# google/yggdrasil-decision-forests

Measured on NVIDIA H100. Metric: GBT boosting iters/sec, 10M rows x 200 num feats, higher is better.
Workload: dtype int64 fixed-point sums (q24 gradients), f64 split scores

## Files before the change

yggdrasil-decision-forests_b200/_build.py:

```python
import os
import subprocess

HERE = os.path.dirname(os.path.abspath(__file__))
CSRC = os.path.join(HERE, "csrc")
LIB = os.environ.get("YGG_B200_LIB") or os.path.join(HERE, "libygg_b200.so")
EXTRA_FLAGS = os.environ.get("YGG_B200_NVCC_FLAGS", "").split()
SOURCES = ["ygg_engine.cu", "ygg_dataspec.cc", "ygg_model_io.cc", "ygg_comm.cc", "ygg_binning.cu"]
HEADERS = ["ygg_device.cuh", "ygg_kernels.cuh", "../../include/ygg_b200.h",
           "../../include/ygg_b200_dataspec.h", "../../include/ygg_b200_model.h", "ygg_hist.cuh", "ygg_hist_seg.cuh", "ygg_wide.cuh", "ygg_presort.cuh",
           "../../include/ygg_b200_comm.h", "ygg_internal.h"]

NVCC_FLAGS = [
    "-gencode", "arch=compute_90a,code=sm_90a", "-O3", "-lineinfo", "-std=c++17",
    "-Xcompiler", "-fPIC", "-shared", "-ldl",
]


def _nvcc():
    for cand in (os.environ.get("NVCC"), "/usr/local/cuda/bin/nvcc", "nvcc"):
        if cand and (os.path.sep not in cand or os.path.exists(cand)):
            return cand
    return "nvcc"


def stale():
    if not os.path.exists(LIB):
        return True
    t = os.path.getmtime(LIB)
    for f in SOURCES + HEADERS:
        p = os.path.join(CSRC, f)
        if os.path.exists(p) and os.path.getmtime(p) > t:
            return True
    return False


def build(force=False, verbose=False):
    if os.environ.get("YGG_B200_LIB") and os.path.exists(LIB) and not force:
        return LIB
    if not force and not stale():
        return LIB
    srcs = [os.path.join(CSRC, s) for s in SOURCES if os.path.exists(os.path.join(CSRC, s))]
    import fcntl
    with open(LIB + ".lock", "w") as lock:
        fcntl.flock(lock, fcntl.LOCK_EX)
        try:
            if not force and not stale():
                return LIB
            tmp = "%s.%d.tmp" % (LIB, os.getpid())
            cmd = [_nvcc()] + NVCC_FLAGS + EXTRA_FLAGS + (["-Xptxas", "-v"] if verbose else []) + ["-o", tmp] + srcs
            subprocess.check_call(cmd)
            os.replace(tmp, LIB)
        finally:
            fcntl.flock(lock, fcntl.LOCK_UN)
    return LIB


if __name__ == "__main__":
    print(build(force=True, verbose=True))
```

yggdrasil-decision-forests_b200/csrc/ygg_engine.cu:

```cuda
#include <algorithm>
#include <mutex>
#include <random>
#include <cmath>
#include <cstdarg>
#include <cstdio>
#include <cstdlib>
#include <cstring>
#include <limits>
#include <map>
#include <queue>
#include <string>
#include <thread>
#include <vector>

#include <cuda_runtime.h>
#include <cub/device/device_radix_sort.cuh>
#include <cub/device/device_scan.cuh>
#include <nvtx3/nvToolsExt.h>

#include "../../include/ygg_b200.h"
#include "ygg_internal.h"
#include "../../include/ygg_b200_model.h"
#include "ygg_kernels.cuh"
#include "ygg_wide.cuh"
// ... 43 lines not shown
  if (static_cast<int>(done.size()) <= device) done.resize(device + 1, 0);
  if (done[device]) return;
  cudaMemPool_t pool;
  if (cudaDeviceGetDefaultMemPool(&pool, device) == cudaSuccess) {
    unsigned long long threshold = ~0ull;
    cudaMemPoolSetAttribute(pool, cudaMemPoolAttrReleaseThreshold, &threshold);
  }
  cudaGetLastError();
  done[device] = 1;
}

template <typename T>
int dev_alloc(T** p, size_t count) {
  int device = 0;
  cudaGetDevice(&device);
  configure_pool_once(device);
  const size_t bytes = std::max<size_t>(count, 1) * sizeof(T);
  YGG_CUDA(cudaMallocAsync(reinterpret_cast<void**>(p), bytes, nullptr));
  YGG_CUDA(cudaMemsetAsync(*p, 0, bytes, nullptr));
  YGG_CUDA(cudaStreamSynchronize(nullptr));
  return YGG_OK;
}
template <typename T>
int dev_alloc_plain(T** p, size_t count) {
  YGG_CUDA(cudaMalloc(reinterpret_cast<void**>(p), std::max<size_t>(count, 1) * sizeof(T)));
  return YGG_OK;
}
inline void dev_free(void* p) {
  if (p != nullptr) cudaFreeAsync(p, nullptr);
}

struct ProfileSlot {
  double ms = 0;
  int64_t launches = 0;
};

}


struct LossRec {
  double loss_sum;
  unsigned long long correct;
};

enum ShardMode { kShardNone = 0, kShardFeatures = 1, kShardRows = 2 };

struct HistLaunch {
  int mode;
  int G, S;
  int chunk, grid;
  int window, passes;
  int FL, T;
  int SL;
};

struct ygg_gbt {
  ygg_dataset* ds = nullptr;
  ygg_gbt_config cfg{};
  cudaStream_t stream = nullptr;
  bool has_labels = false;
  uint8_t* d_label_u8 = nullptr;
  float* d_label_f32 = nullptr;
  float initial_prediction = 0.f;
  float* d_pred = nullptr;
  float* d_g = nullptr;
  float* d_h = nullptr;
  uint32_t* d_q24 = nullptr;
  uint32_t* d_hq24 = nullptr;
  uint2* d_act = nullptr;
  uint32_t* d_act_h = nullptr;
  int32_t* d_act_count = nullptr;
  int32_t* d_act_sub = nullptr;
  uint32_t* d_root_cnt = nullptr;
  bool root_cnt_valid = false;
  int n_blocks = 0;
  uint16_t* d_node_of_row = nullptr;
  DeviceState* d_st = nullptr;
  LevelDesc* d_levels = nullptr;
  Family* d_fam[2] = {nullptr, nullptr};
  int32_t* d_slot_node[2] = {nullptr, nullptr};
  NodeRec* d_nodes_all = nullptr;
  NodeRec* d_nodes_scratch = nullptr;
  int tree_capacity = 0;
  unsigned long long* d_hist_sum[2] = {nullptr, nullptr};
  uint32_t* d_hist_cnt[2] = {nullptr, nullptr};
  unsigned long long* d_hist_hsum[2] = {nullptr, nullptr};
  Candidate* d_cand = nullptr;
  uint32_t* d_cand_mask = nullptr;
  int64_t wide_total = 0;
  int wide_slots = 0;
  bool counted = false;
  unsigned long long* d_wsum = nullptr;
  uint32_t* d_wcnt = nullptr;
  unsigned long long* d_whsum = nullptr;
  unsigned long long* d_wnode_sum[2] = {nullptr, nullptr};
  uint32_t* d_wnode_cnt[2] = {nullptr, nullptr};
  unsigned long long* d_wnode_hsum[2] = {nullptr, nullptr};
  float* d_wide_thr = nullptr;
  int32_t* d_wide_feature = nullptr;
  int32_t* d_wide_bins = nullptr;
  int set_words = 0;
  int64_t sort_total = 0;
  int64_t* d_sort_off = nullptr;
  int32_t* d_wide_cat = nullptr;
  int32_t* d_wide_na_bin = nullptr;
  uint32_t* d_wide_set = nullptr;
// ... 265 lines not shown
  cudaFuncAttributes fa{};
  YGG_CUDA(cudaFuncGetAttributes(&fa, k_hist<false, kHistPacked>));
  *budget = static_cast<size_t>(optin) - fa.sharedSizeBytes;
  return YGG_OK;
}
constexpr size_t kHist2SmemBudget = 216 * 1024;

int sub_blocks_of(const ygg_gbt* h) { return h->ds->n_pad / kBlockRows >= 512 ? 8 : 1; }
int chunk_max_count(ygg_gbt* h, int chunk_blocks, uint32_t** d_sub, uint32_t* out_max) {
  const int kSubBlocks = sub_blocks_of(h);
  const ygg_dataset* ds = h->ds;
  const int f_count = h->hist_f_end - h->hist_f_begin;
  const int n_blocks = static_cast<int>(ds->n_pad / kBlockRows);
  const int n_subs = (n_blocks + kSubBlocks - 1) / kSubBlocks;
  if (*d_sub == nullptr) {
    YGG_RETURN_IF_ERROR(dev_alloc(d_sub, static_cast<size_t>(n_subs) * f_count * kMaxBins + 1));
    k_sub_counts<<<dim3(n_subs, f_count), 256>>>(ds->d_bins, ds->n, ds->n_pad, h->hist_f_begin, kSubBlocks, *d_sub);
    YGG_RETURN_IF_ERROR(check_launch("k_sub_counts"));
  }
  uint32_t* d_max = *d_sub + static_cast<size_t>(n_subs) * f_count * kMaxBins;
  YGG_CUDA(cudaMemset(d_max, 0, sizeof(uint32_t)));
  const int subs_per_chunk = chunk_blocks / kSubBlocks;
  const int n_chunks = (n_subs + subs_per_chunk - 1) / subs_per_chunk;
  k_chunk_max<<<dim3(n_chunks, f_count), 256>>>(*d_sub, n_subs, subs_per_chunk, d_max);
  YGG_CUDA(cudaMemcpy(out_max, d_max, sizeof(uint32_t), cudaMemcpyDeviceToHost));
  return YGG_OK;
}

int raise_hist_smem_caps_once(int device) {
  static std::mutex mu;
  static std::vector<char> done;
  std::lock_guard<std::mutex> lock(mu);
  if (static_cast<int>(done.size()) <= device) done.resize(device + 1, 0);
  if (done[device]) return YGG_OK;
  size_t budget = 0;
  YGG_RETURN_IF_ERROR(hist_smem_budget(device, &budget));
  auto set_cap = [](size_t bytes) {
    return [bytes](auto kern) -> int {
      YGG_CUDA(cudaFuncSetAttribute(kern, cudaFuncAttributeMaxDynamicSharedMemorySize, static_cast<int>(bytes)));
      return YGG_OK;
    };
  };
  for (const bool hess : {false, true})
    for (const int mode : {kHistRootSum, kHistPacked, kHistShared})
      for (const bool multi : {false, true}) YGG_RETURN_IF_ERROR(for_hist_kernel(hess, mode, set_cap(budget), multi));
  const auto cap2 = set_cap(kHist2SmemBudget);
  YGG_RETURN_IF_ERROR(cap2(k_hist2<32, true>)); YGG_RETURN_IF_ERROR(cap2(k_hist2<32, false>));
  YGG_RETURN_IF_ERROR(cap2(k_hist2<16, true>)); YGG_RETURN_IF_ERROR(cap2(k_hist2<16, false>));
  YGG_RETURN_IF_ERROR(cap2(k_hist2<8, true>)); YGG_RETURN_IF_ERROR(cap2(k_hist2<8, false>));
  YGG_RETURN_IF_ERROR(set_cap(seg_smem_bytes(64))(k_hist_seg<32, 2>));
  YGG_RETURN_IF_ERROR(set_cap(seg_smem_bytes(32))(k_hist_seg<32, 1>));
  YGG_RETURN_IF_ERROR(set_cap(seg_smem_bytes(16))(k_hist_seg<16, 1>));
  YGG_RETURN_IF_ERROR(set_cap(seg_smem_bytes(8))(k_hist_seg<8, 1>));
  YGG_CUDA(cudaFuncSetAttribute(k_hist_seg<32, 2>, cudaFuncAttributePreferredSharedMemoryCarveout, cudaSharedmemCarveoutMaxShared));
  YGG_CUDA(cudaFuncSetAttribute(k_hist_seg<32, 1>, cudaFuncAttributePreferredSharedMemoryCarveout, cudaSharedmemCarveoutMaxShared));
  YGG_CUDA(cudaFuncSetAttribute(k_hist_seg<16, 1>, cudaFuncAttributePreferredSharedMemoryCarveout, cudaSharedmemCarveoutMaxShared));
  YGG_CUDA(cudaFuncSetAttribute(k_hist_seg<8, 1>, cudaFuncAttributePreferredSharedMemoryCarveout, cudaSharedmemCarveoutMaxShared));
  done[device] = 1;
  return YGG_OK;
}

int configure_launches(ygg_gbt* h) {
  (void)cudaGetLastError();
  const bool hh = hist_hess(h);
  size_t budget = 0;
  YGG_RETURN_IF_ERROR(hist_smem_budget(h->ds->device, &budget));
  YGG_RETURN_IF_ERROR(raise_hist_smem_caps_once(h->ds->device));
  const int f_count = h->hist_f_end - h->hist_f_begin;
  const int n_blocks = static_cast<int>(h->ds->n_pad / kBlockRows);
  const int kSubBlocks = sub_blocks_of(h);
  const double min_items = 1.0, min_items2 = 0.9;
  auto choose_chunk = [&](int n_fgroups, int grid, int step, double need) {
    const int max_c = std::max(step, kHistMaxChunkBlocks / step * step);
    const int min_chunks = std::max(1, (n_blocks + max_c - 1) / max_c);
    int best = max_c;
    double best_score = -1;
    for (int nc = min_chunks; nc <= std::max(min_chunks, n_blocks); nc++) {
      const int c = std::min(max_c, ((n_blocks + nc - 1) / nc + step - 1) / step * step);
      const int real_nc = (n_blocks + c - 1) / c;
      const double per_cta = static_cast<double>(real_nc) * n_fgroups / grid;
      if (per_cta > 8.0 && nc > min_chunks) break;
      const double fill = static_cast<double>(n_blocks) / (static_cast<double>(real_nc) * c);
      const double eff = per_cta / std::ceil(per_cta) * fill;
      const double score = eff + (per_cta >= need ? 0.08 : 0.0);
      if (score > best_score + 1e-9) { best_score = score; best = c; }
    }
    return best;
  };
  const int g_begin = h->hist_f_begin / 4, n_groups = (h->hist_f_end + 3) / 4 - g_begin;
  const char* env_hist2 = std::getenv("YGG_HIST2");
  const bool want_hist2 = env_hist2 != nullptr && std::atoi(env_hist2) != 0;
  HistLaunch khist_plan[32]{};
  for (int l = 0; l < h->num_levels; l++) {
    HistLaunch& pl = h->hist_plan[l];
    pl.mode = hh ? kHistShared : (l == 0 && !sampling(h)) ? kHistRootSum : kHistPacked;
    int S = level_slot_bound(h, l);
    pl.window = 0;
    pl.passes = 1;
    if (hist_smem_bytes(1, S, hh, pl.mode) > budget) {
      if (S > 254)
        return set_error(YGG_ERR_UNIMPLEMENTED, "max_depth=%d needs %d histogram slots at level %d; the active lists carry 8-bit slots",
                         h->cfg.max_depth, S, l);
      int s_pass = 1;
      while (hist_smem_bytes(1, 2 * s_pass + 1, hh, pl.mode) <= budget) s_pass *= 2;
      pl.window = s_pass;
      pl.passes = (S + s_pass - 1) / s_pass;
      S = s_pass + 1;
    }
    int G = 1;
    while (G < 8 && G < f_count && hist_smem_bytes(G + 1, S, hh, pl.mode) <= budget) G++;
    pl.G = G;
    pl.S = S;
    pl.grid = h->ds->num_sms;
    pl.FL = pl.T = 0;
    if (want_hist2 && !hh && S <= 2 && (l > 0 || pl.mode == kHistRootSum)) {
      int FL = 32;
      while (FL > 8 && FL / 2 >= 4 * n_groups) FL /= 2;
      int T = 2;
      if (hist2_smem_bytes(FL, S, T, l == 0) > kHist2SmemBudget) T = 1;
      if (hist2_smem_bytes(FL, S, T, l == 0) <= kHist2SmemBudget) { pl.FL = FL; pl.T = T; }
    }
    const bool packed = pl.mode == kHistPacked || (pl.FL > 0 && l > 0);
    const int n_fgroups = pl.FL > 0 ? (n_groups + pl.FL / 4 - 1) / (pl.FL / 4) : (f_count + G - 1) / G;
    pl.chunk = choose_chunk(n_fgroups, pl.grid, packed ? kSubBlocks : 1, pl.FL > 0 ? min_items2 : min_items);
    pl.SL = 0;
    khist_plan[l] = pl;
    const int S_level = level_slot_bound(h, l);
    if (!hh && l > 0 && pl.mode == kHistPacked && pl.FL == 0 && S_level >= seg_min_slots(f_count, h->ds->n)) {
      int SL = 32;
      while (SL > 8 && SL / 2 >= f_count) SL /= 2;
      pl.SL = SL;
      pl.G = 1;
      pl.S = S_level;
      pl.window = 0;
      pl.passes = 1;
      pl.grid = h->ds->num_sms * kSegMinBlocks;
      pl.chunk = std::min(std::max(kSubBlocks, kHistMaxChunkBlocks / kSubBlocks * kSubBlocks),
                          (n_blocks + kSubBlocks - 1) / kSubBlocks * kSubBlocks);
    }
  }
  {
    std::map<int, uint32_t> max_of_chunk;
    uint32_t* d_sub = nullptr;
    int status = YGG_OK;
    for (int l = 0; l < h->num_levels && status == YGG_OK; l++) {
      HistLaunch& pl = h->hist_plan[l];
      if (pl.mode != kHistPacked && (pl.FL == 0 || l == 0)) continue;
      int chunk = pl.chunk;
      while (chunk >= kSubBlocks) {
        auto it = max_of_chunk.find(chunk);
        if (it == max_of_chunk.end()) {
          uint32_t m = 0;
          status = chunk_max_count(h, chunk, &d_sub, &m);
          if (status != YGG_OK) break;
          it = max_of_chunk.emplace(chunk, m).first;
        }
        if (it->second <= kPackedMaxUpdates) break;
        const int smaller = static_cast<int>(static_cast<double>(chunk) * 0.9 * kPackedMaxUpdates / it->second) / kSubBlocks * kSubBlocks;
        const int next = std::min(smaller, chunk - kSubBlocks);
        chunk = (next < kSubBlocks && chunk > kSubBlocks) ? kSubBlocks : next;
      }
      if (chunk < kSubBlocks) {
        if (pl.SL > 0) pl = khist_plan[l];
        pl.mode = kHistShared;
        pl.FL = 0;
        pl.chunk = choose_chunk((f_count + pl.G - 1) / pl.G, pl.grid, 1, min_items);
      } else {
        pl.chunk = chunk;
      }
    }
    dev_free(d_sub);
    if (status != YGG_OK) return status;
  }
  h->part_smem_children = static_cast<int>((32 * 1024) / (kPartWords * sizeof(uint32_t)));
  return YGG_OK;
}
// ... 302 lines not shown
    YGG_RETURN_IF_ERROR(dev_alloc(&h->d_hseg_blk, ranges));
    YGG_RETURN_IF_ERROR(dev_alloc(&h->d_hseg_off, ranges + 1));
    YGG_RETURN_IF_ERROR(dev_alloc(&h->d_hseg_piece, ranges + 1));
    YGG_RETURN_IF_ERROR(dev_alloc(&h->d_hseg_meta, 4));
    size_t temp_bytes = 0;
    YGG_CUDA(cub::DeviceScan::InclusiveSum(nullptr, temp_bytes, h->d_hseg_blk, h->d_hseg_blk, static_cast<int>(ranges)));
    char* temp = nullptr;
    YGG_RETURN_IF_ERROR(dev_alloc(&temp, temp_bytes));
    h->hseg_temp_bytes = temp_bytes;
    h->d_hseg_temp = temp;
    return YGG_OK;
  };
  const int st = alloc_all();
  if (st != YGG_OK) free_seg_buffers(h);
  return st;
}

int launch_hist_seg(ygg_gbt* h, int l, const LevelBuf& lb, const LevelDesc* levels, const HistLaunch& pl) {
  ygg_dataset* ds = h->ds;
  YGG_RETURN_IF_ERROR(ensure_bins_rows(ds));
  YGG_RETURN_IF_ERROR(ensure_seg_buffers(h));
  const int f_count = h->hist_f_end - h->hist_f_begin;
  const int n_chunks = (h->n_blocks + pl.chunk - 1) / pl.chunk;
  const int fpl = seg_lane_features(pl.SL, f_count);
  const int n_fg = seg_feature_groups(pl.SL, fpl, h->hist_f_begin, f_count);
  const int target_pieces = std::max(1, (kSegItemsPerCta * pl.grid + n_fg - 1) / n_fg);
  k_seg_count<<<std::min(h->n_blocks, ds->num_sms * 8), 256, 0, h->stream>>>(h->d_act, h->d_act_count, h->n_blocks, pl.S,
                                                                               levels, l, h->d_hseg_blk);
  YGG_RETURN_IF_ERROR(check_launch("k_seg_count"));
  YGG_CUDA(cub::DeviceScan::InclusiveSum(h->d_hseg_temp, h->hseg_temp_bytes, h->d_hseg_blk, h->d_hseg_blk, pl.S * h->n_blocks,
                                         h->stream));
  k_seg_ranges<<<1, kSegScanThreads, 0, h->stream>>>(h->d_hseg_blk, pl.S, h->n_blocks, pl.chunk, n_chunks, target_pieces,
                                                     h->d_hseg_off, h->d_hseg_piece, h->d_hseg_meta);
  YGG_RETURN_IF_ERROR(check_launch("k_seg_ranges"));
  k_seg_scatter<<<std::min(h->n_blocks, ds->num_sms * 8), 256, 0, h->stream>>>(h->d_act, h->d_act_count, h->n_blocks, pl.S, levels, l,
                                                               h->d_hseg_blk, h->d_hseg);
  YGG_RETURN_IF_ERROR(check_launch("k_seg_scatter"));
  SegParams sp{};
  sp.rows = ds->d_bins_rows; sp.row_bytes = static_cast<uint32_t>(seg_row_bytes(ds->F));
  sp.seg = h->d_hseg; sp.seg_off = h->d_hseg_off; sp.piece_start = h->d_hseg_piece; sp.meta = h->d_hseg_meta;
  sp.n_ranges = pl.S * n_chunks; sp.n_chunks = n_chunks;
  sp.f_begin = h->hist_f_begin; sp.f_count = f_count;
  sp.hist_sum = lb.sum; sp.hist_cnt = lb.cnt;
  sp.f_chunk = lb.f_chunk; sp.chunk_stride = static_cast<long long>(lb.chunk_u64);
  const size_t smem = seg_smem_bytes(pl.SL * fpl);
  if (fpl == 2) k_hist_seg<32, 2><<<pl.grid, kSegThreads, smem, h->stream>>>(sp);
  else if (pl.SL == 32) k_hist_seg<32, 1><<<pl.grid, kSegThreads, smem, h->stream>>>(sp);
  else if (pl.SL == 16) k_hist_seg<16, 1><<<pl.grid, kSegThreads, smem, h->stream>>>(sp);
  else k_hist_seg<8, 1><<<pl.grid, kSegThreads, smem, h->stream>>>(sp);
  h->launches_total += 5;
  return check_launch("k_hist_seg");
}

int ensure_root_counts(ygg_gbt* h) {
  if (h->root_cnt_valid) return YGG_OK;
  const int f_count = h->hist_f_end - h->hist_f_begin;
  if (h->d_root_cnt) dev_free(h->d_root_cnt);
  h->d_root_cnt = nullptr;
  const LevelBuf lb = level_buf(h, 1, 1);
  const size_t padded = static_cast<size_t>(lb.W) * lb.f_chunk * kMaxBins;
  YGG_RETURN_IF_ERROR(dev_alloc(&h->d_root_cnt, padded));
  YGG_CUDA(cudaMemsetAsync(h->d_root_cnt, 0, padded * sizeof(uint32_t), h->stream));
  dim3 grid(std::max(1, h->ds->num_sms * 8 / std::max(1, f_count)), f_count);
  k_root_counts<<<grid, 256, 0, h->stream>>>(h->ds->d_bins, h->ds->n, h->ds->n_pad, f_count, h->hist_f_begin, h->d_root_cnt);
  h->launches_total++;
  YGG_RETURN_IF_ERROR(check_launch("k_root_counts"));
  h->root_cnt_valid = true;
  return YGG_OK;
}

int accumulate_level(ygg_gbt* h, int l, const LevelBuf& lb, const LevelDesc* levels, const HistLaunch& pl) {
  const ygg_dataset* ds = h->ds;
  const int hist_f_count = h->hist_f_end - h->hist_f_begin;
  YGG_RETURN_IF_ERROR(zero_planes(h, lb));
  if (pl.mode == kHistRootSum) {
    const size_t row = static_cast<size_t>(lb.f_chunk) * kMaxBins * sizeof(uint32_t);
    YGG_CUDA(cudaMemcpy2DAsync(lb.cnt, lb.chunk_u64 * sizeof(unsigned long long), h->d_root_cnt, row, row, lb.W,
                               cudaMemcpyDeviceToDevice, h->stream));
  }
  if (pl.SL > 0) return launch_hist_seg(h, l, lb, levels, pl);
  if (pl.FL > 0) {
    YGG_RETURN_IF_ERROR(ensure_bins4(h->ds));
    Hist2Params hp{};
    hp.bins4 = ds->d_bins4; hp.n_pad = ds->n_pad; hp.n = ds->n; hp.q24 = h->d_q24; hp.act = h->d_act;
    hp.act_count = h->d_act_count; hp.act_sub = h->d_act_sub; hp.n_blocks = h->n_blocks;
    hp.f_begin = h->hist_f_begin; hp.f_count = hist_f_count;
    hp.g_begin = h->hist_f_begin / 4; hp.n_groups = (h->hist_f_end + 3) / 4 - hp.g_begin;
    hp.S = pl.S; hp.T = pl.T; hp.chunk_blocks = pl.chunk;
    hp.level = l; hp.levels = levels;
    hp.hist_sum = lb.sum; hp.hist_cnt = lb.cnt;
    hp.f_chunk = lb.f_chunk; hp.chunk_stride = static_cast<long long>(lb.chunk_u64);
    return launch_hist2(h, hp, pl.FL, l == 0, pl.grid);
  }
  HistParams hp{};
  hp.bins = ds->d_bins; hp.n_pad = ds->n_pad; hp.act = h->d_act; hp.act_h = h->d_act_h; hp.q24 = h->d_q24;
  hp.act_count = h->d_act_count; hp.n_blocks = h->n_blocks;
  hp.f_begin = h->hist_f_begin; hp.f_count = hist_f_count; hp.G = pl.G; hp.S = pl.S;
  hp.chunk_blocks = pl.chunk;
  hp.level = l; hp.levels = levels;
  hp.hist_sum = lb.sum; hp.hist_cnt = lb.cnt; hp.hist_hsum = lb.hsum;
  hp.f_chunk = lb.f_chunk; hp.chunk_stride = static_cast<long long>(lb.chunk_u64);
  const size_t smem = hist_smem_bytes(pl.G, pl.S, hist_hess(h), pl.mode);
  if (pl.window > 0) {
    for (int pass = 0; pass < pl.passes; pass++) {
      hp.level = l | ((pass * pl.window) << 8) | (pl.window << 20);
      YGG_RETURN_IF_ERROR(launch_hist(h, hp, pl.mode, pl.grid, smem, true));
    }
    return YGG_OK;
  }
  return launch_hist(h, hp, pl.mode, pl.grid, smem);
}

int do_allreduce(ygg_gbt* h, void* buf, int64_t count, int dtype, int op) {
  if (h->allreduce == nullptr) return set_error(YGG_ERR_INVALID_ARGUMENT, "row sharding without an all-reduce function");
  const int rc = h->allreduce(h->exchange_ctx, buf, count, dtype, op, h->stream);
  if (rc != 0) return set_error(YGG_ERR_CUDA, "all-reduce failed with code %d", rc);
  return YGG_OK;
}

int launch_weight_sums(ygg_gbt* h, NodeRec* nodes) {
  ProfScope ps(h, "select");
  WeightSumParams wp{};
  wp.n = h->ds->n; wp.node_of_row = h->d_node_of_row; wp.selected = sampling(h) ? h->d_selected : nullptr;
  wp.weight = h->d_weight; wp.g2w = h->cur_g2w != nullptr ? h->cur_g2w : h->d_g2w; wp.st = h->d_st; wp.w_pow2 = h->w_pow2; wp.nodes = nodes;
  wp.sums = h->d_wsums; wp.levels = h->d_levels; wp.num_levels = h->num_levels + 1;
  wp.smem_nodes = h->max_nodes <= 2048 ? h->max_nodes : 0;
  YGG_CUDA(cudaMemsetAsync(h->d_wsums, 0, static_cast<size_t>(h->max_nodes) * 2 * sizeof(unsigned long long), h->stream));
  const size_t smem = static_cast<size_t>(wp.smem_nodes) * 2 * sizeof(unsigned long long);
  k_weight_sums_rows<<<h->ds->num_sms * 4, 256, smem, h->stream>>>(wp);
  if (h->shard_mode == kShardRows)
    YGG_RETURN_IF_ERROR(do_allreduce(h, h->d_wsums, static_cast<int64_t>(h->max_nodes) * 2, 1, 0));
  k_weight_sums_finish<<<1, 1024, 0, h->stream>>>(wp);
  h->launches_total += 2;
// ... 2317 lines not shown
  return st;
}

int ygg_gbt_set_predictions(ygg_gbt* h, const float* pred, int64_t n) {
  if (!h || !pred) return set_error(YGG_ERR_INVALID_ARGUMENT, "null argument");
  if (h->dart) return set_error(YGG_ERR_UNIMPLEMENTED, "DART keeps its own accumulator of the predictions: not combined with ygg_gbt_set_predictions");
  if (n != h->ds->n) return set_error(YGG_ERR_INVALID_ARGUMENT, "n mismatch");
  YGG_CUDA(cudaSetDevice(h->ds->device));
  YGG_RETURN_IF_ERROR(apply_pending(h));
  YGG_CUDA(cudaMemcpyAsync(h->d_pred, pred, n * sizeof(float), cudaMemcpyHostToDevice, h->stream));
  YGG_CUDA(cudaStreamSynchronize(h->stream));
  return YGG_OK;
}

int ygg_tree_train_on_gradients(ygg_gbt* h, const float* gradients, const float* hessians, ygg_node* out,
                                int32_t capacity, int32_t* n_nodes) {
  if (!h || !gradients || !out || !n_nodes) return set_error(YGG_ERR_INVALID_ARGUMENT, "null argument");
  if (weighted(h)) return set_error(YGG_ERR_UNIMPLEMENTED, "ygg_tree_train_on_gradients takes unit gradients; not combined with example weights");
  if (has_h(h) && !hessians) return set_error(YGG_ERR_INVALID_ARGUMENT, "hessians required for this loss");
  YGG_CUDA(cudaSetDevice(h->ds->device));
  (void)cudaGetLastError();
  YGG_RETURN_IF_ERROR(apply_pending(h));
  const int64_t n = h->ds->n;
  YGG_CUDA(cudaMemcpyAsync(h->d_g, gradients, n * sizeof(float), cudaMemcpyHostToDevice, h->stream));
  if (has_h(h)) YGG_CUDA(cudaMemcpyAsync(h->d_h, hessians, n * sizeof(float), cudaMemcpyHostToDevice, h->stream));
  const int root_candidate = (n >= h->cfg.min_examples && 1 < h->cfg.max_depth) ? 1 : 0;
  k_begin_iteration<<<1, 1, 0, h->stream>>>(h->d_st, h->d_levels, h->d_fam[0], h->d_slot_node[0], root_candidate);
  h->launches_total++;
  k_absmax<<<elementwise_grid(h), 256, 0, h->stream>>>(h->d_g, n, h->d_st);
  h->launches_total++;
  YGG_RETURN_IF_ERROR(check_launch("k_absmax"));
  h->scratch_tree = false;
  YGG_RETURN_IF_ERROR(grow_tree(h, h->d_nodes_scratch));
  if (h->cfg.growing_strategy == 1) YGG_RETURN_IF_ERROR(best_first_prune(h, h->d_nodes_scratch));
  YGG_RETURN_IF_ERROR(check_device_error(h));
  h->scratch_tree = true;
  std::vector<ygg_node> flat;
  YGG_RETURN_IF_ERROR(fetch_tree(h, h->d_nodes_scratch, &flat, true));
  *n_nodes = static_cast<int32_t>(flat.size());
  if (static_cast<int32_t>(flat.size()) > capacity) return set_error(YGG_ERR_INVALID_ARGUMENT, "capacity %d < %zu nodes", capacity, flat.size());
  std::memcpy(out, flat.data(), flat.size() * sizeof(ygg_node));
  return YGG_OK;
}

int ygg_debug_hist_plan(const ygg_gbt* h, int32_t level, ygg_hist_plan* out) {
  if (!h || !out) return set_error(YGG_ERR_INVALID_ARGUMENT, "null argument");
  if (level < 0 || level >= h->num_levels) return set_error(YGG_ERR_INVALID_ARGUMENT, "level %d outside [0, %d)", level, h->num_levels);
  const HistLaunch& pl = h->hist_plan[level];
  ygg_hist_plan p{};
  if (pl.FL > 0) {
    p.mode = YGG_HIST_HIST2; p.group = pl.FL; p.hist2_tiles = pl.T;
  } else if (pl.SL > 0) {
    p.mode = YGG_HIST_SEGMENTED; p.group = pl.SL;
  } else {
    p.mode = pl.mode == kHistRootSum ? YGG_HIST_ROOT_SUM : pl.mode == kHistPacked ? YGG_HIST_PACKED : YGG_HIST_SHARED;
    p.group = pl.G;
  }
  p.chunk_blocks = pl.chunk;
  p.slot_window = pl.window;
  p.grid = pl.grid;
  *out = p;
  return YGG_OK;
}

int ygg_debug_level_histogram(ygg_gbt* h, int32_t level, const ygg_hist_plan* plan, const float* gradients,
                              const float* second, const int32_t* slot_of_row, int32_t n_slots, uint64_t* out_sum,
                              uint32_t* out_cnt, uint64_t* out_second, float* out_scales) {
  if (!h || !gradients || !slot_of_row || !out_sum || !out_cnt || !out_scales) return set_error(YGG_ERR_INVALID_ARGUMENT, "null argument");
  if (level < 0 || level >= h->num_levels) return set_error(YGG_ERR_INVALID_ARGUMENT, "level %d outside [0, %d)", level, h->num_levels);
  if (n_slots < 1 || n_slots > 254) return set_error(YGG_ERR_INVALID_ARGUMENT, "n_slots=%d outside [1, 254] (8-bit slots)", n_slots);
  const bool hh = hist_hess(h);
  if (hh != (second != nullptr) || hh != (out_second != nullptr))
    return set_error(YGG_ERR_INVALID_ARGUMENT, hh ? "this handle keeps a second histogram plane: `second` and `out_second` are required"
                                                  : "this handle keeps no second histogram plane: `second` and `out_second` must be NULL");
  const float v_pow2 = hh ? (weighted(h) ? h->w_pow2 : h_pow2_of(h)) : 0.f;
  const int64_t n = h->ds->n;
  bool all_slot0 = true;
  for (int64_t r = 0; r < n; r++) {
    if (!std::isfinite(gradients[r])) return set_error(YGG_ERR_INVALID_ARGUMENT, "gradient of row %lld is not finite", static_cast<long long>(r));
    if (hh && !(second[r] >= 0.f && second[r] <= v_pow2))
      return set_error(YGG_ERR_INVALID_ARGUMENT, "second-plane value of row %lld outside [0, %g]", static_cast<long long>(r), v_pow2);
    if (slot_of_row[r] < -1 || slot_of_row[r] >= n_slots)
      return set_error(YGG_ERR_INVALID_ARGUMENT, "slot %d of row %lld outside [-1, %d)", slot_of_row[r], static_cast<long long>(r), n_slots);
    all_slot0 &= slot_of_row[r] == 0;
  }
  HistLaunch pl{};
  if (plan == nullptr) {
    pl = h->hist_plan[level];
    if (n_slots > level_slot_bound(h, level))
      return set_error(YGG_ERR_INVALID_ARGUMENT, "the plan of level %d holds %d slots, %d requested", level, level_slot_bound(h, level), n_slots);
  } else {
    const ygg_hist_plan& p = *plan;
    if (p.mode < YGG_HIST_ROOT_SUM || p.mode > YGG_HIST_SEGMENTED) return set_error(YGG_ERR_INVALID_ARGUMENT, "unknown mode %d", p.mode);
    if (p.chunk_blocks < 1 || p.chunk_blocks > kHistMaxChunkBlocks)
      return set_error(YGG_ERR_INVALID_ARGUMENT, "chunk_blocks=%d outside [1, %d]", p.chunk_blocks, kHistMaxChunkBlocks);
    if (p.grid < 1 || p.grid > 65535) return set_error(YGG_ERR_INVALID_ARGUMENT, "grid=%d outside [1, 65535]", p.grid);
    if (p.slot_window < 0) return set_error(YGG_ERR_INVALID_ARGUMENT, "slot_window=%d", p.slot_window);
    pl.chunk = p.chunk_blocks; pl.grid = p.grid;
    if (p.mode == YGG_HIST_HIST2) {
      if (p.group != 8 && p.group != 16 && p.group != 32) return set_error(YGG_ERR_INVALID_ARGUMENT, "k_hist2: %d feature lanes (8, 16 or 32)", p.group);
      if (p.hist2_tiles != 1 && p.hist2_tiles != 2) return set_error(YGG_ERR_INVALID_ARGUMENT, "k_hist2: %d sub-tiles (1 or 2)", p.hist2_tiles);
      if (p.slot_window != 0) return set_error(YGG_ERR_INVALID_ARGUMENT, "k_hist2 has no multi-pass form");
      if (n_slots > 2) return set_error(YGG_ERR_INVALID_ARGUMENT, "k_hist2 with %d slots (at most 2)", n_slots);
      if (hist2_smem_bytes(p.group, n_slots, p.hist2_tiles, level == 0) > kHist2SmemBudget)
        return set_error(YGG_ERR_INVALID_ARGUMENT, "k_hist2 needs %zu bytes of shared memory (budget 216 KB)", hist2_smem_bytes(p.group, n_slots, p.hist2_tiles, level == 0));
      pl.FL = p.group; pl.T = p.hist2_tiles; pl.S = n_slots; pl.G = 1; pl.passes = 1;
      pl.mode = level == 0 ? kHistRootSum : kHistPacked;
    } else if (p.mode == YGG_HIST_SEGMENTED) {
      if (level == 0) return set_error(YGG_ERR_INVALID_ARGUMENT, "k_hist_seg runs below the root only");
      if (hh) return set_error(YGG_ERR_INVALID_ARGUMENT, "a second histogram plane is accumulated by the shared layout only");
      if (p.group != 8 && p.group != 16 && p.group != 32) return set_error(YGG_ERR_INVALID_ARGUMENT, "k_hist_seg: %d feature lanes (8, 16 or 32)", p.group);
      if (p.slot_window != 0) return set_error(YGG_ERR_INVALID_ARGUMENT, "k_hist_seg has no multi-pass form");
      pl.SL = p.group; pl.S = n_slots; pl.G = 1; pl.passes = 1;
      pl.mode = kHistPacked;
    } else {
      if (p.group < 1 || p.group > 8) return set_error(YGG_ERR_INVALID_ARGUMENT, "k_hist: group=%d outside [1, 8]", p.group);
      pl.mode = p.mode == YGG_HIST_ROOT_SUM ? kHistRootSum : p.mode == YGG_HIST_PACKED ? kHistPacked : kHistShared;
      pl.G = p.group;
      if (p.slot_window > 0) {
        if (pl.mode == kHistRootSum) return set_error(YGG_ERR_INVALID_ARGUMENT, "the root layout has no multi-pass form");
        pl.window = p.slot_window; pl.S = p.slot_window + 1; pl.passes = (n_slots + p.slot_window - 1) / p.slot_window;
      } else {
        pl.S = n_slots; pl.passes = 1;
      }
      size_t budget = 0;
      YGG_RETURN_IF_ERROR(hist_smem_budget(h->ds->device, &budget));
      if (hist_smem_bytes(pl.G, pl.S, hh, pl.mode) > budget)
        return set_error(YGG_ERR_INVALID_ARGUMENT, "k_hist with G=%d and %d slots per pass needs %zu bytes of shared memory (budget %zu)",
                         pl.G, pl.S, hist_smem_bytes(pl.G, pl.S, hh, pl.mode), budget);
    }
  }
  if (hh && (pl.FL > 0 || pl.SL > 0 || pl.mode != kHistShared))
    return set_error(YGG_ERR_INVALID_ARGUMENT, "a second histogram plane is accumulated by the shared layout only");
  if (pl.mode == kHistRootSum && (level != 0 || sampling(h) || !all_slot0 || n_slots != 1))
    return set_error(YGG_ERR_INVALID_ARGUMENT, "the root layouts need level 0, no row sampling and every row in slot 0");
  if (h->wide_total > 0 && n_slots > h->wide_slots)
    return set_error(YGG_ERR_INVALID_ARGUMENT, "the wide-column planes of this handle hold %d slots, %d requested", h->wide_slots, n_slots);
  YGG_CUDA(cudaSetDevice(h->ds->device));
  (void)cudaGetLastError();
  if (pl.mode == kHistPacked) {
    const int sub = sub_blocks_of(h);
    if (pl.chunk % sub != 0)
      return set_error(YGG_ERR_INVALID_ARGUMENT, "packed layout: chunk_blocks=%d is not a multiple of the %d-block sub-chunk", pl.chunk, sub);
    uint32_t* d_sub = nullptr;
    uint32_t m = 0;
    const int st = chunk_max_count(h, pl.chunk, &d_sub, &m);
    dev_free(d_sub);
    YGG_RETURN_IF_ERROR(st);
    if (m > kPackedMaxUpdates)
      return set_error(YGG_ERR_INVALID_ARGUMENT, "packed layout: a bin receives %u rows in one chunk of %d blocks (at most %u)", m, pl.chunk, kPackedMaxUpdates);
  }
  if (pl.mode == kHistRootSum) YGG_RETURN_IF_ERROR(ensure_root_counts(h));
  YGG_RETURN_IF_ERROR(raise_hist_smem_caps_once(h->ds->device));

  const int64_t n_pad = h->ds->n_pad;
  const int f_hist = h->hist_f_end - h->hist_f_begin;
  std::vector<uint8_t> sel(n), slot8(n);
  for (int64_t r = 0; r < n; r++) {
    sel[r] = slot_of_row[r] >= 0 ? 1 : 0;
    slot8[r] = static_cast<uint8_t>(slot_of_row[r] >= 0 ? slot_of_row[r] : 0);
  }
  std::vector<LevelDesc> lv(32, LevelDesc{0, 0, 0, 0});
  lv[level] = LevelDesc{0, n_slots, n_slots, 0};
  const LevelBuf probe = level_buf(h, n_slots, 1);
  float *d_g = nullptr, *d_v = nullptr;
  uint8_t *d_sel = nullptr, *d_slot = nullptr;
  uint16_t* d_nor = nullptr;
  DeviceState* d_st = nullptr;
  LevelDesc* d_lv = nullptr;
  unsigned long long *d_stats = nullptr, *d_buf = nullptr;
  auto run = [&]() -> int {
    YGG_RETURN_IF_ERROR(dev_alloc(&d_g, n));
    if (hh) YGG_RETURN_IF_ERROR(dev_alloc(&d_v, n));
    YGG_RETURN_IF_ERROR(dev_alloc(&d_sel, n));
    YGG_RETURN_IF_ERROR(dev_alloc(&d_slot, n));
    YGG_RETURN_IF_ERROR(dev_alloc(&d_nor, n_pad));
    YGG_RETURN_IF_ERROR(dev_alloc(&d_st, 1));
    YGG_RETURN_IF_ERROR(dev_alloc(&d_lv, lv.size()));
    YGG_RETURN_IF_ERROR(dev_alloc(&d_stats, 3));
    YGG_RETURN_IF_ERROR(dev_alloc(&d_buf, probe.total_u64));
// ... 491 lines not shown
```

yggdrasil-decision-forests_b200/csrc/ygg_kernels.cuh:

```cuda
#pragma once
#include <cstdint>
#include <cuda_runtime.h>

#include "ygg_device.cuh"
#include "ygg_hist.cuh"
#include "ygg_hist2.cuh"

namespace ygg {

__device__ __forceinline__ unsigned long long warp_sum_u64(unsigned long long v) {
#pragma unroll
  for (int o = 16; o > 0; o >>= 1) v += __shfl_xor_sync(0xffffffffu, v, o);
  return v;
}
__device__ __forceinline__ double warp_sum_f64(double v) {
#pragma unroll
  for (int o = 16; o > 0; o >>= 1) v += __shfl_xor_sync(0xffffffffu, v, o);
  return v;
}

__device__ __forceinline__ float pow2_cover(unsigned int max_bits) {
  if (max_bits == 0u) return 1.f;
  const int e = static_cast<int>(max_bits >> 23) - 127;
  const bool exact = (max_bits & 0x7FFFFFu) == 0u;
  return exact ? exp2f(static_cast<float>(e)) : exp2f(static_cast<float>(e + 1));
}

constexpr int kLossParts = 4096;
struct LossPartials {
  double loss[kLossParts];
  unsigned long long correct[kLossParts];
  unsigned int done;
};
__device__ __forceinline__ void reduce_loss_in_order(LossPartials* part, double loss, unsigned long long correct, double* out_loss,
                                                     unsigned long long* out_correct) {
  __shared__ bool s_last;
  __shared__ double s_l[256];
  __shared__ unsigned long long s_c[256];
  if (threadIdx.x == 0) {
    part->loss[blockIdx.x] = loss;
    part->correct[blockIdx.x] = correct;
    __threadfence();
    s_last = atomicInc(&part->done, gridDim.x - 1) == gridDim.x - 1;
  }
  __syncthreads();
  if (!s_last) return;
  __threadfence();
  double l = 0;
  unsigned long long c = 0;
  for (unsigned int i = threadIdx.x; i < gridDim.x; i += 256) {
    l += reinterpret_cast<volatile double*>(part->loss)[i];
    c += reinterpret_cast<volatile unsigned long long*>(part->correct)[i];
  }
  s_l[threadIdx.x] = l;
  s_c[threadIdx.x] = c;
  __syncthreads();
  if (threadIdx.x == 0) {
    for (int i = 1; i < 256; i++) { l += s_l[i]; c += s_c[i]; }
    *out_loss = l;
// ... 1571 lines not shown
```

Before: 163.9.

## Add TMA-pipelined 32-feature-lane root histogram kernel with carry-split 64-bit sums

Adds a dedicated root-level histogram kernel, k_hist_root. It streams 32 feature columns plus the q24 gradients per 1024-row tile into shared memory with a 4-stage bulk-copy/mbarrier pipeline. Each lane owns one feature and accumulates 32-bit low words with shared atomics, detecting carries to bump a separate high word, which avoids 64-bit shared atomics. The planner selects it at level 0 in root-sum mode when at least 32 features are present and the shared memory fits. The trade-off is a large 1024-thread, one-block-per-SM footprint and more complex flushing to the global histogram.

```diff
diff --git a/yggdrasil-decision-forests_b200/_build.py b/yggdrasil-decision-forests_b200/_build.py
--- a/yggdrasil-decision-forests_b200/_build.py
+++ b/yggdrasil-decision-forests_b200/_build.py
@@ -7,7 +7,7 @@
 EXTRA_FLAGS = os.environ.get("YGG_B200_NVCC_FLAGS", "").split()
 SOURCES = ["ygg_engine.cu", "ygg_dataspec.cc", "ygg_model_io.cc", "ygg_comm.cc", "ygg_binning.cu"]
 HEADERS = ["ygg_device.cuh", "ygg_kernels.cuh", "../../include/ygg_b200.h",
-           "../../include/ygg_b200_dataspec.h", "../../include/ygg_b200_model.h", "ygg_hist.cuh", "ygg_hist_seg.cuh", "ygg_wide.cuh", "ygg_presort.cuh",
+           "../../include/ygg_b200_dataspec.h", "../../include/ygg_b200_model.h", "ygg_hist.cuh", "ygg_hist_root.cuh", "ygg_hist_seg.cuh", "ygg_wide.cuh", "ygg_presort.cuh",
            "../../include/ygg_b200_comm.h", "ygg_internal.h"]
 
 NVCC_FLAGS = [
diff --git a/yggdrasil-decision-forests_b200/csrc/ygg_engine.cu b/yggdrasil-decision-forests_b200/csrc/ygg_engine.cu
--- a/yggdrasil-decision-forests_b200/csrc/ygg_engine.cu
+++ b/yggdrasil-decision-forests_b200/csrc/ygg_engine.cu
@@ -119,6 +119,7 @@
   int window, passes;
   int FL, T;
   int SL;
+  int RL;
 };
 
 struct ygg_gbt {
@@ -490,6 +491,7 @@
   YGG_RETURN_IF_ERROR(set_cap(seg_smem_bytes(32))(k_hist_seg<32, 1>));
   YGG_RETURN_IF_ERROR(set_cap(seg_smem_bytes(16))(k_hist_seg<16, 1>));
   YGG_RETURN_IF_ERROR(set_cap(seg_smem_bytes(8))(k_hist_seg<8, 1>));
+  YGG_RETURN_IF_ERROR(set_cap(hist_root_smem_bytes())(k_hist_root));
   YGG_CUDA(cudaFuncSetAttribute(k_hist_seg<32, 2>, cudaFuncAttributePreferredSharedMemoryCarveout, cudaSharedmemCarveoutMaxShared));
   YGG_CUDA(cudaFuncSetAttribute(k_hist_seg<32, 1>, cudaFuncAttributePreferredSharedMemoryCarveout, cudaSharedmemCarveoutMaxShared));
   YGG_CUDA(cudaFuncSetAttribute(k_hist_seg<16, 1>, cudaFuncAttributePreferredSharedMemoryCarveout, cudaSharedmemCarveoutMaxShared));
@@ -558,8 +560,12 @@
       if (hist2_smem_bytes(FL, S, T, l == 0) > kHist2SmemBudget) T = 1;
       if (hist2_smem_bytes(FL, S, T, l == 0) <= kHist2SmemBudget) { pl.FL = FL; pl.T = T; }
     }
+    pl.RL = 0;
+    if (l == 0 && pl.mode == kHistRootSum && pl.FL == 0 && f_count >= kHistRootMinFeatures && hist_root_smem_bytes() <= budget)
+      pl.RL = kRootLanes;
     const bool packed = pl.mode == kHistPacked || (pl.FL > 0 && l > 0);
-    const int n_fgroups = pl.FL > 0 ? (n_groups + pl.FL / 4 - 1) / (pl.FL / 4) : (f_count + G - 1) / G;
+    const int n_fgroups = pl.FL > 0 ? (n_groups + pl.FL / 4 - 1) / (pl.FL / 4)
+                          : pl.RL > 0 ? hist_root_groups(f_count) : (f_count + G - 1) / G;
     pl.chunk = choose_chunk(n_fgroups, pl.grid, packed ? kSubBlocks : 1, pl.FL > 0 ? min_items2 : min_items);
     pl.SL = 0;
     khist_plan[l] = pl;
@@ -968,6 +974,18 @@
   return check_launch("k_hist_seg");
 }
 
+int launch_hist_root(ygg_gbt* h, const LevelBuf& lb, const HistLaunch& pl) {
+  HistParams hp{};
+  hp.bins = h->ds->d_bins; hp.n_pad = h->ds->n_pad; hp.q24 = h->d_q24; hp.n_blocks = h->n_blocks;
+  hp.f_begin = h->hist_f_begin; hp.f_count = h->hist_f_end - h->hist_f_begin;
+  hp.chunk_blocks = pl.chunk;
+  hp.hist_sum = lb.sum;
+  hp.f_chunk = lb.f_chunk; hp.chunk_stride = static_cast<long long>(lb.chunk_u64);
+  k_hist_root<<<pl.grid, kRootThreads, hist_root_smem_bytes(), h->stream>>>(hp);
+  h->launches_total++;
+  return check_launch("k_hist_root");
+}
+
 int ensure_root_counts(ygg_gbt* h) {
   if (h->root_cnt_valid) return YGG_OK;
   const int f_count = h->hist_f_end - h->hist_f_begin;
@@ -995,6 +1013,7 @@
                                cudaMemcpyDeviceToDevice, h->stream));
   }
   if (pl.SL > 0) return launch_hist_seg(h, l, lb, levels, pl);
+  if (pl.RL > 0) return launch_hist_root(h, lb, pl);
   if (pl.FL > 0) {
     YGG_RETURN_IF_ERROR(ensure_bins4(h->ds));
     Hist2Params hp{};
@@ -3418,6 +3437,8 @@
     p.mode = YGG_HIST_HIST2; p.group = pl.FL; p.hist2_tiles = pl.T;
   } else if (pl.SL > 0) {
     p.mode = YGG_HIST_SEGMENTED; p.group = pl.SL;
+  } else if (pl.RL > 0) {
+    p.mode = YGG_HIST_ROOT_SUM; p.group = pl.RL;
   } else {
     p.mode = pl.mode == kHistRootSum ? YGG_HIST_ROOT_SUM : pl.mode == kHistPacked ? YGG_HIST_PACKED : YGG_HIST_SHARED;
     p.group = pl.G;
@@ -3480,9 +3501,12 @@
       pl.SL = p.group; pl.S = n_slots; pl.G = 1; pl.passes = 1;
       pl.mode = kHistPacked;
     } else {
-      if (p.group < 1 || p.group > 8) return set_error(YGG_ERR_INVALID_ARGUMENT, "k_hist: group=%d outside [1, 8]", p.group);
+      const bool root_lanes = p.mode == YGG_HIST_ROOT_SUM && p.group == kRootLanes;
+      if (!root_lanes && (p.group < 1 || p.group > 8))
+        return set_error(YGG_ERR_INVALID_ARGUMENT, "k_hist: group=%d outside [1, 8] (the root layout also takes %d feature lanes)", p.group, kRootLanes);
       pl.mode = p.mode == YGG_HIST_ROOT_SUM ? kHistRootSum : p.mode == YGG_HIST_PACKED ? kHistPacked : kHistShared;
-      pl.G = p.group;
+      pl.G = root_lanes ? 1 : p.group;
+      pl.RL = root_lanes ? kRootLanes : 0;
       if (p.slot_window > 0) {
         if (pl.mode == kHistRootSum) return set_error(YGG_ERR_INVALID_ARGUMENT, "the root layout has no multi-pass form");
         pl.window = p.slot_window; pl.S = p.slot_window + 1; pl.passes = (n_slots + p.slot_window - 1) / p.slot_window;
@@ -3491,7 +3515,9 @@
       }
       size_t budget = 0;
       YGG_RETURN_IF_ERROR(hist_smem_budget(h->ds->device, &budget));
-      if (hist_smem_bytes(pl.G, pl.S, hh, pl.mode) > budget)
+      if (root_lanes && hist_root_smem_bytes() > budget)
+        return set_error(YGG_ERR_INVALID_ARGUMENT, "k_hist_root needs %zu bytes of shared memory (budget %zu)", hist_root_smem_bytes(), budget);
+      if (!root_lanes && hist_smem_bytes(pl.G, pl.S, hh, pl.mode) > budget)
         return set_error(YGG_ERR_INVALID_ARGUMENT, "k_hist with G=%d and %d slots per pass needs %zu bytes of shared memory (budget %zu)",
                          pl.G, pl.S, hist_smem_bytes(pl.G, pl.S, hh, pl.mode), budget);
     }
diff --git a/yggdrasil-decision-forests_b200/csrc/ygg_hist_root.cuh b/yggdrasil-decision-forests_b200/csrc/ygg_hist_root.cuh
--- /dev/null
+++ b/yggdrasil-decision-forests_b200/csrc/ygg_hist_root.cuh
@@ -0,0 +1,165 @@
+#pragma once
+#include <cstdint>
+#include <cuda_runtime.h>
+
+#include "ygg_device.cuh"
+#include "ygg_hist.cuh"
+
+namespace ygg {
+
+constexpr int kRootThreads = 1024;
+constexpr int kRootWarps = kRootThreads / 32;
+constexpr int kRootLanes = 32;
+constexpr int kRootRows = 1024;
+constexpr int kRootStages = 4;
+constexpr int kHistRootMinFeatures = 32;
+constexpr int kRootTilesPerBlock = kBlockRows / kRootRows;
+constexpr uint32_t kRootColBytes = kRootRows + 16;
+constexpr uint32_t kRootStageBytes = kRootLanes * kRootColBytes + kRootRows * 4;
+constexpr uint32_t kRootHistBytes = kMaxBins * 2 * kRootLanes * 4;
+static_assert(kRootRows / 16 % kRootWarps == 0, "every warp takes the same number of 16-row steps of a tile");
+static_assert(kRootTilesPerBlock >= kRootStages, "a work item holds at least kRootStages tiles");
+
+__host__ __device__ inline size_t hist_root_smem_bytes() {
+  return kRootHistBytes + static_cast<size_t>(kRootStages) * kRootStageBytes + kRootStages * 8 + kRootStages * 4;
+}
+__host__ __device__ inline int hist_root_groups(int f_count) { return (f_count + kRootLanes - 1) / kRootLanes; }
+
+__device__ __forceinline__ void smem_ld_v4(uint32_t addr, uint32_t* v) {
+  asm volatile("ld.shared.v4.u32 {%0,%1,%2,%3}, [%4];" : "=r"(v[0]), "=r"(v[1]), "=r"(v[2]), "=r"(v[3]) : "r"(addr));
+}
+
+__device__ __forceinline__ uint32_t shl_carry(uint32_t m, uint32_t old, uint32_t q) {
+  uint32_t r;
+  asm("{\n\t.reg .u32 t;\n\tadd.cc.u32 t, %1, %2;\n\taddc.u32 %0, %3, %3;\n\t}" : "=r"(r) : "r"(old), "r"(q), "r"(m));
+  return r;
+}
+
+__global__ void __launch_bounds__(kRootThreads, 1) k_hist_root(HistParams p) {
+  extern __shared__ __align__(128) uint8_t smem_raw[];
+  uint32_t* hist = reinterpret_cast<uint32_t*>(smem_raw);
+  uint32_t s_hist = static_cast<uint32_t>(__cvta_generic_to_shared(smem_raw));
+  asm volatile("mov.u32 %0, %0;" : "+r"(s_hist));
+  const uint32_t s_tiles = s_hist + kRootHistBytes;
+  const uint32_t s_full = s_tiles + kRootStages * kRootStageBytes;
+  int* s_release = reinterpret_cast<int*>(smem_raw + kRootHistBytes + kRootStages * kRootStageBytes + kRootStages * 8);
+
+  const int tid = threadIdx.x, lane = tid & 31, warp = tid >> 5;
+  const int n_fg = hist_root_groups(p.f_count);
+  const int n_chunks = (p.n_blocks + p.chunk_blocks - 1) / p.chunk_blocks;
+  const int n_items = n_chunks * n_fg;
+  if (static_cast<int>(blockIdx.x) >= n_items) return;
+
+  auto item_tiles = [&](int item) {
+    const int b0 = item / n_fg * p.chunk_blocks;
+    return min(p.chunk_blocks, p.n_blocks - b0) * kRootTilesPerBlock;
+  };
+  auto group_of = [&](int item, int* f0, int* gcount) {
+    const int fg = item % n_fg;
+    *f0 = fg * p.f_count / n_fg;
+    *gcount = (fg + 1) * p.f_count / n_fg - *f0;
+  };
+  auto issue = [&](int item, int t, uint32_t s) {
+    int f0, gcount;
+    group_of(item, &f0, &gcount);
+    const int64_t row0 = static_cast<int64_t>(item / n_fg) * p.chunk_blocks * kBlockRows + static_cast<int64_t>(t) * kRootRows;
+    const uint32_t bar = s_full + 8 * s, stage = s_tiles + s * kRootStageBytes;
+    if (lane == 0) mbar_expect_tx(bar, static_cast<uint32_t>(gcount + 4) * kRootRows);
+    __syncwarp();
+    asm volatile("fence.proxy.async.shared::cta;" ::: "memory");
+    if (lane < gcount)
+      tma_bulk_g2s(stage + lane * kRootColBytes, p.bins + static_cast<int64_t>(p.f_begin + f0 + lane) * p.n_pad + row0, kRootRows, bar);
+    if (lane == 31) tma_bulk_g2s(stage + kRootLanes * kRootColBytes, p.q24 + row0, kRootRows * 4, bar);
+  };
+  auto advance = [&](int* item, int* t) {
+    *t += kRootStages;
+    while (*item < n_items && *t >= item_tiles(*item)) {
+      *t -= item_tiles(*item);
+      *item += gridDim.x;
+    }
+  };
+
+  if (tid == 0) {
+    for (int s = 0; s < kRootStages; s++) mbar_init(s_full + 8 * s, 1);
+    fence_barrier_init();
+  }
+  if (tid < kRootStages) s_release[tid] = 0;
+  for (int i = tid; i < static_cast<int>(kRootHistBytes / 16); i += kRootThreads)
+    reinterpret_cast<uint4*>(hist)[i] = make_uint4(0u, 0u, 0u, 0u);
+  __syncthreads();
+  if (warp == 0) {
+    for (int s = 0; s < kRootStages; s++) issue(blockIdx.x, s, s);
+  }
+
+  const uint32_t lane4 = static_cast<uint32_t>(lane) * 4u, lane_hist = s_hist + lane4;
+  constexpr uint32_t kBinBytes = 2u * kRootLanes * 4u, kCarryBytes = kRootLanes * 4u;
+  uint32_t g = 0;
+  for (int item = blockIdx.x; item < n_items; item += gridDim.x) {
+    const int n_tiles = item_tiles(item);
+    for (int t = 0; t < n_tiles; t++, g++) {
+      const uint32_t s = g % kRootStages;
+      mbar_wait(s_full + 8 * s, (g / kRootStages) & 1u);
+      const uint32_t stage = s_tiles + s * kRootStageBytes;
+      const uint32_t col = stage + static_cast<uint32_t>(lane) * kRootColBytes;
+      const uint32_t qrow = stage + kRootLanes * kRootColBytes;
+#pragma unroll 1
+      for (int k = warp; k < kRootRows / 16; k += kRootWarps) {
+        uint32_t b[4];
+        smem_ld_v4(col + k * 16u, b);
+        uint32_t cm = 0;
+#pragma unroll
+        for (int h = 0; h < 2; h++) {
+          uint32_t q[8], a[8], old[8];
+          smem_ld_v4(qrow + k * 64u + h * 32u, q);
+          smem_ld_v4(qrow + k * 64u + h * 32u + 16u, q + 4);
+#pragma unroll
+          for (int j = 0; j < 8; j++) a[j] = __byte_perm(b[2 * h + j / 4], lane4, 0x5504u | ((j & 3) << 4));
+#pragma unroll
+          for (int j = 0; j < 8; j++) old[j] = smem_add(s_hist + a[j], q[j]);
+#pragma unroll
+          for (int j = 0; j < 8; j++) cm = shl_carry(cm, old[j], q[j]);
+        }
+        while (cm != 0u) {
+          const int bit = 31 - __clz(cm);
+          const int j = 15 - bit;
+          const uint32_t w = (j & 8) ? ((j & 4) ? b[3] : b[2]) : ((j & 4) ? b[1] : b[0]);
+          smem_red(lane_hist + ((w >> ((j & 3) * 8)) & 0xFFu) * kBinBytes + kCarryBytes, 1u);
+          cm &= ~(1u << bit);
+        }
+      }
+      __syncwarp();
+      int before = 0;
+      if (lane == 0) before = atomicAdd(&s_release[s], 1);
+      before = __shfl_sync(0xFFFFFFFFu, before, 0);
+      if (before == static_cast<int>((g / kRootStages + 1) * kRootWarps) - 1) {
+        int ni = item, nt = t;
+        advance(&ni, &nt);
+        if (ni < n_items) issue(ni, nt, s);
+      }
+    }
+    __syncthreads();
+
+    int f0, gcount;
+    group_of(item, &f0, &gcount);
+    const int tr = lane >> 2, tq = lane & 3;
+    for (int tile = warp; tile < kMaxBins / 8 * (kRootLanes / 16); tile += kRootWarps) {
+      const int bin = (tile >> 1) * 8 + tr;
+      const int c0 = ((tile & 1) * 4 + tq) * 4;
+      uint4* w = reinterpret_cast<uint4*>(hist + bin * 2 * kRootLanes + c0);
+      const uint4 lo4 = w[0], hi4 = w[kRootLanes / 4];
+      w[0] = make_uint4(0u, 0u, 0u, 0u);
+      w[kRootLanes / 4] = make_uint4(0u, 0u, 0u, 0u);
+      const uint32_t los[4] = {lo4.x, lo4.y, lo4.z, lo4.w}, his[4] = {hi4.x, hi4.y, hi4.z, hi4.w};
+#pragma unroll
+      for (int j = 0; j < 4; j++) {
+        const unsigned long long sum = (static_cast<unsigned long long>(his[j]) << 32) + los[j];
+        if (c0 + j >= gcount || sum == 0ull) continue;
+        size_t oc;
+        atomicAdd(&p.hist_sum[slot_hist_offset(0, f0 + c0 + j, bin, p.f_chunk, p.chunk_stride, &oc)], sum);
+      }
+    }
+    __syncthreads();
+  }
+}
+
+}
diff --git a/yggdrasil-decision-forests_b200/csrc/ygg_kernels.cuh b/yggdrasil-decision-forests_b200/csrc/ygg_kernels.cuh
--- a/yggdrasil-decision-forests_b200/csrc/ygg_kernels.cuh
+++ b/yggdrasil-decision-forests_b200/csrc/ygg_kernels.cuh
@@ -5,6 +5,7 @@
 #include "ygg_device.cuh"
 #include "ygg_hist.cuh"
 #include "ygg_hist2.cuh"
+#include "ygg_hist_root.cuh"
 
 namespace ygg {
 
```

Measured after the change: 167.2 (median of 6 runs). 2.0% higher.
